# hpsim/OGL

Hardware: AMD Instinct MI355X
Metric: cg_iters_per_sec (higher is better)
Workload: dtype f64

## Files before the change

ogl_amd/csrc/kernels.hpp:

```cpp
#pragma once
#include <hip/hip_runtime.h>

#include "common.hpp"

namespace ogl {

struct DevCriterion {
    double tolerance, rel_tol;
    int32_t min_iter, max_iter, frequency, export_res;
};

struct DevScalars {
    double rho, prev_rho, beta;
    double alpha, omega, gamma;
    double norm_factor;
    double init_res, res;
    double xbar;
    double sums[4];
    int32_t iter;
    int32_t stop;
    int32_t n_evals;
    int32_t stop_phase;
    int32_t stop_turn;
    int32_t comm_error;
// ... 224 lines not shown
void launch_cg_rho_norm(hipStream_t st, int32_t n, const double *r, const double *inv_diag,
                        double *part_rho, double *part_norm, const DevScalars *gate);
void launch_cg_step1(hipStream_t st, int32_t n, double *p, const double *r, const double *inv_diag,
                     const DevScalars *s);
void launch_cg_step2(hipStream_t st, int32_t n, double *x, double *r, const double *p,
                     const double *q, const double *inv_diag, double *part_rho, double *part_norm,
                     const DevScalars *s);

struct HaloPutFused;
void launch_cg_step1x(hipStream_t st, int32_t n, double *p, double *x, const double *r,
                      const double *inv_diag, const DevScalars *s, const HaloPutFused *put = nullptr);
void launch_cg_step2r(hipStream_t st, int32_t n, double *r, const double *q, const double *inv_diag,
                      double *part_rho, double *part_norm, const DevScalars *s, double *z_out = nullptr,
                      const HaloPutFused *put = nullptr);

void launch_cg_step1x_fin(hipStream_t st, int32_t n, double *p, double *x, const double *r, const double *inv_diag,
                          const DevScalars *sin, DevScalars *sout, const double *part_rho,
                          const double *part_norm, double *history, int first, const LeadBox &lead = LeadBox{},
                          double *p_out = nullptr, const PRing &ring = PRing{});
void launch_cg_step2r_fin(hipStream_t st, int32_t n, double *r, const double *q, const double *inv_diag,
                          double *part_rho, double *part_norm, const DevScalars *sin, DevScalars *sout,
                          const double *part_beta, double *z_out = nullptr,
                          const LeadBox &lead = LeadBox{});
constexpr int FUSED_FIN_MAX_CHUNKS = 1024;
void launch_cg_turn_sym(hipStream_t st, const DevSym &A, const double *p_in, double *p_out, double *x, const double *z,
                        double *q, double *part_beta, const DevScalars *sin, DevScalars *sout,
                        const double *part_rho, const double *part_norm, double *history, int first,
                        const LeadBox &lead = LeadBox{});
void launch_cg_turn_sym_big(hipStream_t st, const DevSym &A, const double *p_in, double *p_out, double *x,
                            const double *z, double *q, double *part_beta, const DevScalars *s,
                            const HaloFused &hf = HaloFused{}, const double *p_halo_in = nullptr,
                            double *p_halo_out = nullptr);

void launch_gmres_mgs_fold(hipStream_t st, int32_t n, double *w, const double *vprev, double *h_out, const double *vdot,
                           const double *part_in, double *part_out, const DevScalars *gate, const LeadBox &lead = LeadBox{},
                           uint32_t tag = 0);
void launch_bicg_fold1(hipStream_t st, int32_t n, double *p, const double *r, const double *v, const double *inv_diag,
                       double *y, const DevScalars *sin, DevScalars *sout, const double *part_rho,
                       const double *part_norm, double *history, const LeadBox &lead = LeadBox{});
void launch_bicg_fold2(hipStream_t st, int32_t n, const double *r, const double *v, double *sv, const double *inv_diag,
                       double *z, double *part_norm_out, const DevScalars *sin, DevScalars *sout,
                       const double *part_beta, const LeadBox &lead = LeadBox{});
void launch_bicg_fold3(hipStream_t st, int32_t n, double *x, double *r, const double *sv, const double *t,
                       const double *y, const double *z, const double *rr, double *part_rho_out, double *part_norm_out,
                       const DevScalars *sin, DevScalars *sout, const double *part_gamma, const double *part_tt,
                       const double *part_snorm, double *history, int turn, const LeadBox &lead = LeadBox{});
// ... 107 lines not shown
```

ogl_amd/csrc/kernels_krylov.hip:

```cpp
#include "device_common.hpp"

namespace ogl {

namespace {

__global__ __launch_bounds__(BLOCK) void k_scale(int n, double *__restrict__ v, double f)
{
    const int i = blockIdx.x * BLOCK + threadIdx.x;
    if (i < n) v[i] = v[i] * f;
}

__global__ __launch_bounds__(BLOCK) void k_fill_xbar(int n, double *__restrict__ v,
                                                     const DevScalars *s)
{
    const int i = blockIdx.x * BLOCK + threadIdx.x;
    if (i < n) v[i] = s->xbar;
}

enum PartialOp { P_SUM = 0, P_DOT = 1, P_NORM1 = 2 };
template <int OP>
__global__ __launch_bounds__(BLOCK) void k_partials(int n, int n_chunks,
                                                    const double *__restrict__ a,
                                                    const double *__restrict__ b,
                                                    double *__restrict__ part,
// ... 480 lines not shown
        double2 vz = vrh;
        if (inv_diag) {
            vz.x = vrh.x * vi[h].x;
            vz.y = vrh.y * vi[h].y;
        }
        if (z_out) st2(z_out, rh, vz);
        double d = 0.0, a = 0.0;
        if (rh.n > 0) {
            d += vrh.x * vz.x;
            a += fabs(vrh.x);
        }
        if (rh.n > 1) {
            d += vrh.y * vz.y;
            a += fabs(vrh.y);
        }
        block_sum2(d, a, slot);
        if (threadIdx.x == 0) {
            part_rho[chunk] = d;
            part_norm[chunk] = a;
        }
    }
}

__global__ __launch_bounds__(BLOCK) void k_bicg_step1(int n, double *__restrict__ p,
                                                      const double *__restrict__ r,
                                                      const double *__restrict__ v,
                                                      const double *__restrict__ inv_diag,
                                                      double *__restrict__ y, const DevScalars *s)
{
    if (s->stop) return;
    const double rho = s->rho, prev = s->prev_rho, alpha = s->alpha, omega = s->omega;
    const RowPair rp = my_rows(blockIdx.x, n);
    const double2 vr = ld2_stream(r, rp);
    double2 vp = vr;
    if (prev * omega != 0.0) {
        const double tmp = rho / prev * alpha / omega;
        const double2 po = ld2_stream(p, rp), vv = ld2_stream(v, rp);
        vp.x = vr.x + tmp * (po.x - omega * vv.x);
        vp.y = vr.y + tmp * (po.y - omega * vv.y);
    }
    if (inv_diag) st2_stream(p, rp, vp); else st2(p, rp, vp);
    if (inv_diag) {
        const double2 vi = ld2_stream(inv_diag, rp);
        double2 vy;
        vy.x = vp.x * vi.x;
        vy.y = vp.y * vi.y;
// ... 847 lines not shown
    if (led) {
        OGL_STEP1X_K(true)
    } else {
        OGL_STEP1X(false, 0);
    }
#undef OGL_STEP1X_K
#undef OGL_STEP1X
}

constexpr int STEP2R_LEAD_CPW = 2;
void launch_cg_step2r_fin(hipStream_t st, int32_t n, double *r, const double *q, const double *inv_diag,
                          double *part_rho, double *part_norm, const DevScalars *sin, DevScalars *sout,
                          const double *part_beta, double *z_out, const LeadBox &lead)
{
    const int nc = (int)n_chunks(n);
    if (nc == 0) return;
    if (lead.box && nc >= 3 * FIN_WAVES)
        hipLaunchKernelGGL((k_cg_step2r_fin<true, STEP2R_LEAD_CPW>), dim3((nc + STEP2R_LEAD_CPW - 1) / STEP2R_LEAD_CPW),
                           dim3(BLOCK), 0, st, n, r, q, inv_diag, part_rho, part_norm, sin, sout, part_beta, nc, z_out, lead);
    else
        hipLaunchKernelGGL((k_cg_step2r_fin<false, 1>), dim3(nc), dim3(BLOCK), 0, st, n, r, q, inv_diag, part_rho, part_norm,
                           sin, sout, part_beta, nc, z_out, LeadBox{});
}

void launch_cg_step2(hipStream_t st, int32_t n, double *x, double *r, const double *p,
                     const double *q, const double *inv_diag, double *part_rho, double *part_norm,
                     const DevScalars *s)
{
    const int nc = (int)n_chunks(n);
    if (nc == 0) return;
    hipLaunchKernelGGL(k_cg_step2, dim3(nc), dim3(BLOCK), 0, st, n, x, r, p, q, inv_diag, part_rho,
                       part_norm, s);
}

void launch_bicg_step1(hipStream_t st, int32_t n, double *p, const double *r, const double *v,
                       const double *inv_diag, double *y, const DevScalars *s)
{
    const int nc = (int)n_chunks(n);
    if (nc == 0) return;
    hipLaunchKernelGGL(k_bicg_step1, dim3(nc), dim3(BLOCK), 0, st, n, p, r, v, inv_diag, y, s);
}

void launch_bicg_step2(hipStream_t st, int32_t n, const double *r, const double *v, double *sv,
                       const double *inv_diag, double *z, double *part_norm, const DevScalars *s)
{
    const int nc = (int)n_chunks(n);
// ... 174 lines not shown
```

ogl_amd/csrc/launch_key.hpp:

```cpp
#pragma once
#include <cstdint>
#include <cstring>
#include <type_traits>

#include "kernels.hpp"

namespace ogl {

struct KeyHasher {
    uint64_t h = 1469598103934665603ull;
    void bytes(const void *p, size_t n)
    {
        const unsigned char *c = static_cast<const unsigned char *>(p);
        for (size_t i = 0; i < n; ++i) h = (h ^ c[i]) * 1099511628211ull;
    }
    template <class T>
    std::enable_if_t<std::is_arithmetic<T>::value || std::is_pointer<T>::value || std::is_enum<T>::value> operator()(const T &v)
    {
        bytes(&v, sizeof(v));
    }
};

#define OGL_VIEW_FIELDS(T, n)                                                                                        \
    static_assert(sizeof(T) == n, "a field of " #T " was added, removed or resized: bring visit(KeyHasher &, const " #T \
// ... 11 lines not shown
    h(a.n_rows), h(a.width), h(a.stride), h(a.cols), h(a.vals), h(a.stream);
}
OGL_VIEW_FIELDS(DevSell, 112);
inline void visit(KeyHasher &h, const DevSell &a)
{
    h(a.n_rows), h(a.chunks), h(a.dict), h(a.codes), h(a.vals), h(a.spill_chunk_ptr), h(a.spill_rows), h(a.spill_ptrs);
    h(a.spill_cols), h(a.spill_vals), h(a.stream), h(a.xcd_group), h(a.rmap), h(a.block_order), h(a.n_blocks);
}
OGL_VIEW_FIELDS(DevSym, 64);
inline void visit(KeyHasher &h, const DevSym &a)
{
    h(a.n_rows), h(a.nd);
    for (int j = 0; j < 4; ++j) h(a.d[j]);
    h(a.mask), h(a.planes), h(a.stream), h(a.block_order), h(a.n_blocks);
}
OGL_VIEW_FIELDS(DevSymx, 96);
inline void visit(KeyHasher &h, const DevSymx &a)
{
    h(a.n_rows), h(a.chunks), h(a.chunks_general), h(a.n_blocks_general), h(a.mask), h(a.planes), h(a.ex_rowptr), h(a.ex_cols);
    h(a.ex_lrow), h(a.ex_vals), h(a.stream), h(a.fast), h(a.xcd_group), h(a.n_blocks);
}
OGL_VIEW_FIELDS(LeadBox, 24);
inline void visit(KeyHasher &h, const LeadBox &a) { h(a.box), h(a.timeout_ticks), h(a.early_loads); }

#undef OGL_VIEW_FIELDS

}
```

ogl_amd/csrc/solver.cpp:

```cpp
#include "solver_internal.hpp"

#include "setup_kernels.hpp"

#include <algorithm>
#include <atomic>
#include <chrono>
#include <condition_variable>
#include <cmath>
#include <cstddef>
#include <cstring>
#include <future>
#if defined(__x86_64__)
#include <immintrin.h>
#endif
#include <sched.h>
#include <mutex>
#include <thread>

using namespace ogl;


namespace {
#if defined(__x86_64__)
__attribute__((target("avx2"))) void stream_copy_avx2(char *d, const char *s, size_t len)
// ... 186 lines not shown
        (void)hipStreamSynchronize(comm_stream);
        stream_destroy(comm_stream);
        ev_destroy(ev_packed);
        ev_destroy(ev_received);
    }
    if (own_stream && stream) stream_destroy(stream);
}

void ogl_solver::drop_cg_graph()
{
    if (cg_graph) {
        (void)hipGraphExecDestroy(cg_graph);
        ledger::destroyed(ledger::GRAPH_EXEC);
    }
    cg_graph = nullptr;
    cg_graph_key = 0;
}

ogl_solver::~ogl_solver()
{
    drop_cg_graph();
    ledger::pinned_free(h_scal);
    ledger::dev_free(lead_box);
    for (auto &e : poll_ev)
        if (e) ev_destroy(e);
    for (auto &e : prof_ev)
        if (e) ev_destroy(e);
    for (auto &e : chk_ev)
        if (e) ev_destroy(e);
}

double ogl_solver::prop(const std::string &key, double dflt) const
{
    auto it = props.find(key);
    return it == props.end() ? dflt : it->second;
}

double ogl_solver::stream_above_bytes() const
{
    static const double env_default = [] {
        const char *e = std::getenv("OGL_STREAM_ABOVE_BYTES");
        return e ? atof(e) : STREAM_MATRIX_ABOVE_BYTES;
    }();
    return prop("streamAboveBytes", env_default);
}

// ... 988 lines not shown
```

ogl_amd/csrc/solver.hpp:

```cpp
#pragma once
#include <hip/hip_runtime.h>

#include <algorithm>
#include <map>
#include <memory>
#include <string>
#include <vector>

#include "comm.hpp"
#include "common.hpp"
#include "host_matrix.hpp"
#include "kernels.hpp"
#include "setup_kernels.hpp"
#include "spmv_layouts.hpp"

namespace ogl {

struct PrecondData {
    int kind = 0;
    size_t n_rows = 0;
    int stride = 0;
    int32_t n_blocks = 0;
    bool uniform_blocks = false;
    bool through_perm = false;
// ... 165 lines not shown
    ogl::DevBuf<double> d_p_halo;
    ogl::DevBuf<double> d_bj_tmp0, d_bj_tmp1;
    ogl::DevBuf<double> d_v, d_s, d_t, d_y, d_z, d_rr;
    ogl::DevBuf<double> d_V, d_gm;
    ogl::DevBuf<double> d_isai_tmp;
    ogl::DevBuf<double> d_fac_tmp[3];
    bool precond_ready = false;
    uint64_t precond_serial = 0, precond_pat = 0;
    bool precond_current() const;
    std::vector<int32_t> fac_seg_fwd, fac_seg_bwd;
    ogl::DevBuf<double> d_part0, d_part1, d_part2;
    int64_t band_order_rows = 0;
    bool source_diag_valid = false;
    int64_t csr_band_rows = 0;
    uint64_t csr_band_pat = 0;
    int csr_band(int64_t *band);
    ogl::DevBuf<int32_t> d_band_order;
    ogl::DevBuf<double> d_part3, d_part4, d_part5;
    ogl::DevBuf<ogl::DevScalars> d_scal;
    ogl::DevBuf<double> d_history;
    ogl::DevScalars *h_scal = nullptr;
    hipEvent_t poll_ev[2] = {nullptr, nullptr};
    unsigned long long *lead_box = nullptr;
    hipEvent_t chk_ev[2] = {nullptr, nullptr};
    bool x_resident = false, b_resident = false;
    ogl::PrecondData own_precond;
    const ogl::PrecondData *precond_data = nullptr;
    const double *precond = nullptr;

    std::map<std::string, double> props;

    std::vector<double> history;
    double t_update_matrix_ms = 0;
    std::vector<hipEvent_t> prof_ev;

    ~ogl_solver();

    int set_matrix(const ogl_ldu_view &ldu);
    int solve(const double *source, double *psi, ogl_perf *perf);
    int apply_resident(ogl_perf *perf);
    int upload_vec(ogl::DevBuf<double> &dst, const double *src);
    int ensure_vectors();
    int init_preconditioner();
    int generate_preconditioner(ogl::PrecondData &P);
    void apply_factor(const double *in, double *out, const ogl::DevScalars *gate, double *dot_part);
    int check_factor_breakdown(int32_t word);
    void apply_preconditioner(const double *in, double *out, const ogl::DevScalars *gate,
                              double *dot_part = nullptr);
    int dist_spmv(int mode, const double *x, const double *b, double *y, const ogl::SpmvDots &dots,
                  const ogl::DevScalars *gate, bool prepacked = false);
    void spmv_on(ogl::SpmvLayout l, int mode, const double *x, const double *b, double *y, const ogl::SpmvDots &dots,
                 const ogl::DevScalars *gate, const ogl::HaloFused &hf = ogl::HaloFused{});
    int finalize(int phase, ogl::FinArgs &a);
    int run_cg(ogl_perf *perf);
    int run_bicgstab(ogl_perf *perf);
    int run_krylov(ogl_perf *perf);
    struct KrylovRun;
    int krylov_plan(KrylovRun &k);
    int krylov_prepare(KrylovRun &k);
    int krylov_loop(KrylovRun &k);
    int krylov_enqueue(KrylovRun &k, int count);
    int krylov_finish(KrylovRun &k, ogl_perf *perf);
    int gmres_restart(KrylovRun &k, const ogl::DevScalars *gate);
    int gmres_update_x(KrylovRun &k, int cols, const ogl::DevScalars *gate);
    int turn_gmres(KrylovRun &k, int enq, int pe);
    int turn_cg_generic(KrylovRun &k, int enq, int pe);
    int turn_cg_generic_led(KrylovRun &k, int enq, int pe);
    int turn_cg_two_launch(KrylovRun &k, int enq, int pe);
    int turn_cg_three_launch(KrylovRun &k, int enq, int pe);
    int turn_cg_merged(KrylovRun &k, int enq, int pe);
    int turn_cg_five_launch(KrylovRun &k, int enq, int pe);
    int turn_bicg_folded(KrylovRun &k, int enq, int pe);
    int turn_bicg(KrylovRun &k, int enq, int pe);
    int time_spmv(int repeats, double *avg_ms);
    ogl::DevHalo halo() const;
    double prop(const std::string &key, double dflt) const;
    const ogl_solver *share_from = nullptr;
    const double *offdiag_upper = nullptr, *offdiag_lower = nullptr;
    uint64_t offdiag_sum = 0;
    bool offdiag_valid = false;
    const ogl_label *seen_lower_addr = nullptr, *seen_upper_addr = nullptr;
    ogl_label seen_faces = -1;
    struct SeenIface {
        const ogl_label *face_cells;
        ogl_label size, kind, neighb_proc, neighb_patch;
    };
    std::vector<SeenIface> seen_iface_cells;
    bool saw_addressing(const ogl_ldu_view &ldu) const;
    bool peer_safe_wait() const;
    double stream_above_bytes() const;
    double turn_extra_bytes() const;
    int32_t xcd_group() const;
// ... 3 lines not shown
```

ogl_amd/csrc/solver_krylov.cpp:

```cpp
#include "launch_key.hpp"
#include "solver_internal.hpp"

#include <algorithm>
#include <cmath>
#include <cstring>
#include <vector>

using namespace ogl;

HaloPutFused ogl_solver::begin_halo_put()
{
    HaloPutFused put;
    if (!(pat.non_local_nnz > 0 && peer_halo) || prop("haloFused", 1.0) == 0.0 || peer_safe_wait())
        return put;
    if (++halo_seq == 0) ++halo_seq;
    cur_halo = peer_halo_args(halo_seq);
    put.P = cur_halo;
    put.chunk_sptr = d_chunk_sptr.p;
    put.send_pos = d_send_pos.p;
    put.send_idxs = d_send_idxs.p;
    put.ticket = d_ticket.p;
    put.n_put_chunks = n_put_chunks;
    return put;
}
// ... 128 lines not shown
    int cur = 0;
    bool bicg = false, gmres = false, generic = false, multi = false;
    bool fused = false, fused2 = false, merged = false, merged_halo = false, bicg_fold = false, gmres_fold = false;
    int m = 0;
    int64_t ldv = 0;
    double n_global = 0.0;
    size_t n_halo = 0;
    double *p0 = nullptr, *p1 = nullptr, *ph = nullptr;
    double *z_kept = nullptr;
    LeadBox lead{};
    uint32_t lead_tag = 0;
    DevCriterion crit{};
    bool is_final = false;
    int max_checks = 0, max_turns = 0;
    int prof_stride = 0, prof_cap = 0;
    hipEvent_t ev_chk[2] = {nullptr, nullptr};
    double t_start = 0.0;
    FinArgs fg{}, chk{}, f1{}, f2{};
    const double *beta_ptr = nullptr;
    double *gm = nullptr, *gm_y = nullptr;
    double *y = nullptr, *z = nullptr;
    int enq = 0;
    double *gm_h(int i, int j) const { return gm + (size_t)j * (m + 1) + i; }
    PRing ring{};
    double *p_of_turn(int turn) const
    {
        if (ring.k > 0) return ring.b[turn % ring.k];
        return (merged && (turn & 1)) ? p1 : p0;
    }
    PRing ring_of_turn(int turn) const
    {
        PRing r = ring;
        r.phase = ring.k > 0 ? turn % ring.k : 0;
        return r;
    }
    double *p_halo_of_turn(int turn) const { return ph + (size_t)(turn & 1) * n_halo; }
    bool gmres_scale_late() const { return gmres && !generic && has_diag; }
    bool has_diag = false;
    bool folded() const { return fused || bicg_fold; }
};

int ogl_solver::run_cg(ogl_perf *perf) { return run_krylov(perf); }
int ogl_solver::run_bicgstab(ogl_perf *perf) { return run_krylov(perf); }

int ogl_solver::run_krylov(ogl_perf *perf)
{
// ... 74 lines not shown
    DevScalars *s = k.s;
    const bool bicg = k.bicg, gmres = k.gmres, generic = k.generic, merged = k.merged;
    int ring_k = 0;
    if (k.lead.box != nullptr && k.fused && !k.fused2 && prop("deferX2", 1.0) != 0.0) {
        const double want = prop("deferX", 2.0);
        ring_k = want >= 8.0 ? 8 : want >= 4.0 ? 4 : want >= 2.0 ? 2 : 0;
    }
    props["deferXInUse"] = (double)ring_k;
    props["deferX2InUse"] = ring_k ? 1.0 : 0.0;
    if (merged || ring_k) OGL_TRY(d_p2.alloc((size_t)n + 2, st));
    for (int i = 2; i < ring_k; ++i) OGL_TRY(d_pring[i - 2].alloc((size_t)n + 2, st));
    if (merged && precond) OGL_TRY(d_z.alloc((size_t)n + 2, st));
    k.n_halo = (size_t)pat.non_local_nnz;
    if (k.merged_halo) {
        OGL_TRY(d_p_halo.alloc(2 * k.n_halo + 2, st));
        OGL_HIP_CHECK(hipMemsetAsync(d_p_halo.p, 0, d_p_halo.n * sizeof(double), st));
    }
    k.p0 = d_p.p;
    k.p1 = d_p2.p;
    k.ring.k = ring_k;
    for (int i = 0; i < ring_k; ++i) k.ring.b[i] = i == 0 ? d_p.p : i == 1 ? d_p2.p : d_pring[i - 2].p;
    k.ph = d_p_halo.p;
    k.z_kept = merged && precond ? d_z.p : nullptr;

    k.is_final = cfg.rel_tol == 0.0;
    const int prev_iters = (int)prop(k.is_final ? "prevSolveIters_final" : "prevSolveIters", 1);
    const double prev_cost = prop("_prev_solve", 0.0);
    DevCriterion &crit = k.crit;
    crit.tolerance = cfg.tolerance;
    crit.rel_tol = cfg.rel_tol;
    crit.max_iter = bicg ? 2 * cfg.max_iter : cfg.max_iter;
    crit.export_res = cfg.export_res;
    ogl_host_adapt_criterion(&cfg, prev_iters, prev_cost, &crit.min_iter, &crit.frequency);
    if (crit.frequency < 1) return fail(OGL_ERR_INVALID, "evalFrequency must be >= 1");
    k.max_checks = std::max(crit.max_iter, crit.min_iter) + crit.frequency + 1;
    k.max_turns = bicg ? k.max_checks / 2 + 1 : k.max_checks;
    OGL_TRY(d_history.alloc((size_t)std::max(k.max_checks, crit.max_iter + std::max(1, cfg.norm_eval_limit) + 1) + 4, st));
    if (cfg.export_res)
        OGL_HIP_CHECK(hipMemsetAsync(d_history.p, 0, d_history.n * sizeof(double), st));
    if (k.bicg_fold) {
        OGL_TRY(d_part3.alloc((size_t)nc, st));
        OGL_TRY(d_part4.alloc((size_t)nc, st));
        OGL_TRY(d_part5.alloc((size_t)nc, st));
    }
    if (bicg) {
        const size_t nv = (size_t)n + 2;
// ... 232 lines not shown
    if (enq == 0) OGL_HIP_CHECK(hipEventRecord(k.ev_chk[0], st));
    if (pe >= 0) OGL_HIP_CHECK(hipEventRecord(prof_ev[2 * pe], st));
    launch_cg_turn_sym(st, sym(), k.p_of_turn(enq), k.p_of_turn(enq + 1), d_x.p, k.z_kept ? k.z_kept : d_r.p,
                       d_q.p, d_part2.p, k.s, k.s2, d_part0.p, d_part1.p, d_history.p, enq == 0 ? 1 : 0, k.lead);
    if (pe >= 0) OGL_HIP_CHECK(hipEventRecord(prof_ev[2 * pe + 1], st));
    if (enq == 0) OGL_HIP_CHECK(hipEventRecord(k.ev_chk[1], st));
    launch_cg_step2r_fin(st, k.n, d_r.p, d_q.p, precond, d_part0.p, d_part1.p, k.s2, k.s, d_part2.p, k.z_kept, k.lead);
    return OGL_OK;
}

int ogl_solver::turn_cg_three_launch(KrylovRun &k, int enq, int pe)
{
    hipStream_t st = k.st;
    const int n = k.n;
    if (enq == 0) OGL_HIP_CHECK(hipEventRecord(k.ev_chk[0], st));
    double *p_new = k.p_of_turn(enq + 1);
    launch_cg_step1x_fin(st, n, k.p_of_turn(enq), d_x.p, d_r.p, precond, k.s, k.s2, d_part0.p, d_part1.p, d_history.p,
                         enq == 0 ? 1 : 0, k.lead, p_new, k.ring_of_turn(enq));
    if (enq == 0) OGL_HIP_CHECK(hipEventRecord(k.ev_chk[1], st));
    if (pe >= 0) OGL_HIP_CHECK(hipEventRecord(prof_ev[2 * pe], st));
    OGL_TRY(dist_spmv(SPMV_PLAIN, p_new, nullptr, d_q.p, SpmvDots{p_new, d_part2.p, nullptr}, k.s2));
    if (pe >= 0) OGL_HIP_CHECK(hipEventRecord(prof_ev[2 * pe + 1], st));
    launch_cg_step2r_fin(st, n, d_r.p, d_q.p, precond, d_part0.p, d_part1.p, k.s2, k.s, d_part2.p, nullptr, k.lead);
    return OGL_OK;
}

int ogl_solver::turn_cg_merged(KrylovRun &k, int enq, int pe)
{
    hipStream_t st = k.st;
    const int n = k.n;
    DevScalars *s = k.s;
    if (pe >= 0) OGL_HIP_CHECK(hipEventRecord(prof_ev[2 * pe], st));
    if (k.merged_halo) {
        launch_cg_turn_sym_big(st, sym(), k.p_of_turn(enq), k.p_of_turn(enq + 1), d_x.p,
                               k.z_kept ? k.z_kept : d_r.p, d_q.p, d_part0.p, s,
                               halo_fused_args(cur_halo), k.p_halo_of_turn(enq), k.p_halo_of_turn(enq + 1));
    } else {
        launch_cg_turn_sym_big(st, sym(), k.p_of_turn(enq), k.p_of_turn(enq + 1), d_x.p,
                               k.z_kept ? k.z_kept : d_r.p, d_q.p, d_part0.p, s);
    }
    if (pe >= 0) OGL_HIP_CHECK(hipEventRecord(prof_ev[2 * pe + 1], st));
    OGL_TRY(finalize(FIN_BETA, k.f1));
    if (k.merged_halo) {
        const HaloPutFused put = begin_halo_put();
        launch_cg_step2r(st, n, d_r.p, d_q.p, precond, d_part0.p, d_part1.p, s, k.z_kept, &put);
    } else {
// ... 82 lines not shown
                          SpmvDots{d_s.p, d_part0.p, d_part1.p}, s));
        OGL_TRY(finalize(FIN_BICG_OMEGA, f2));
    }
    launch_bicg_step3(st, n, d_x.p, d_r.p, d_s.p, d_t.p, y, z, d_rr.p, d_part0.p,
                      d_part1.p, s, enq);
    OGL_TRY(finalize(FIN_CG_CHECK, k.chk));
    return OGL_OK;
}

int ogl_solver::krylov_enqueue(KrylovRun &k, int count)
{
    for (int i = 0; i < count; ++i, ++k.enq) {
        const int enq = k.enq;
        const bool prof = k.prof_stride && enq % k.prof_stride == 0 && enq / k.prof_stride < k.prof_cap;
        const int pe = prof ? enq / k.prof_stride : -1;
        if (k.gmres)
            OGL_TRY(turn_gmres(k, enq, pe));
        else if (k.bicg)
            OGL_TRY(k.bicg_fold ? turn_bicg_folded(k, enq, pe) : turn_bicg(k, enq, pe));
        else if (k.generic)
            OGL_TRY(k.fused ? turn_cg_generic_led(k, enq, pe) : turn_cg_generic(k, enq, pe));
        else if (k.fused2)
            OGL_TRY(turn_cg_two_launch(k, enq, pe));
        else if (k.fused)
            OGL_TRY(turn_cg_three_launch(k, enq, pe));
        else if (k.merged)
            OGL_TRY(turn_cg_merged(k, enq, pe));
        else
            OGL_TRY(turn_cg_five_launch(k, enq, pe));
    }
    return OGL_OK;
}

int ogl_solver::krylov_loop(KrylovRun &k)
{
    hipStream_t st = k.st;
    const bool fused = k.fused;
    auto poll_record = [&](int slot) -> int {
        OGL_HIP_CHECK(hipMemcpyAsync(&h_scal[slot], k.bicg_fold ? k.slot_s[k.cur] : k.s, sizeof(DevScalars),
                                     hipMemcpyDeviceToHost, st));
        OGL_HIP_CHECK(hipEventRecord(poll_ev[slot], st));
        return OGL_OK;
    };

    const int batch = k.bicg ? 8 : 16;

    const bool graphable = !k.gmres && !k.bicg && !k.generic && !k.multi && k.prof_cap == 0 &&
                           prop("hipGraph", fused ? 1.0 : 0.0) != 0.0;
    auto enqueue_turns = [&](int count) -> int {
        if (!graphable || count != batch || (fused && k.enq == 0)) return krylov_enqueue(k, count);
        KeyHasher kh;
        kh(k.n), kh(batch), kh(cfg.matrix_format), kh(spmv_layout);
        kh(k.fused), kh(k.fused2), kh(k.merged), kh(k.ring.k), kh(k.p0), kh(k.p1), kh(k.z_kept), kh(k.s), kh(k.s2), kh(pat_id);
        for (const void *v : {(const void *)d_p.p, (const void *)d_x.p, (const void *)d_r.p, (const void *)d_q.p,
                              (const void *)precond, (const void *)d_part0.p, (const void *)d_part1.p,
                              (const void *)d_part2.p, (const void *)d_history.p, (const void *)d_z.p, (const void *)d_p2.p})
            kh(v);
        for (int i = 0; i < k.ring.k; ++i) kh((const void *)k.ring.b[i]);
        visit(kh, csr());
        switch (spmv_layout) {
        case SpmvLayout::Ell: visit(kh, ell()); break;
        case SpmvLayout::Sell: visit(kh, sell()); break;
        case SpmvLayout::Sym: visit(kh, sym()); break;
        case SpmvLayout::Symx: visit(kh, symx()); break;
        default: break;
        }
        visit(kh, k.lead);
        const uint64_t key = kh.h;
        if (!cg_graph || key != cg_graph_key) {
            if (cg_graph) {
                (void)hipGraphExecDestroy(cg_graph);
                ledger::destroyed(ledger::GRAPH_EXEC);
            }
            cg_graph = nullptr;
            OGL_HIP_CHECK(hipStreamBeginCapture(st, hipStreamCaptureModeThreadLocal));
            const int before = k.enq;
            const int rc = krylov_enqueue(k, batch);
            k.enq = before;
            hipGraph_t g = nullptr;
            const hipError_t e = hipStreamEndCapture(st, &g);
            if (rc != OGL_OK || e != hipSuccess) {
                if (g) (void)hipGraphDestroy(g);
                return rc != OGL_OK ? rc : fail(OGL_ERR_HIP, "stream capture failed: %s", hipGetErrorString(e));
            }
            const hipError_t ei = hipGraphInstantiate(&cg_graph, g, nullptr, nullptr, 0);
            (void)hipGraphDestroy(g);
            if (ei != hipSuccess) {
                cg_graph = nullptr;
                return fail(OGL_ERR_HIP, "hipGraphInstantiate failed: %s", hipGetErrorString(ei));
            }
// ... 7 lines not shown
    };
    OGL_TRY(enqueue_turns(std::min(batch, k.max_turns - k.enq)));
    OGL_TRY(poll_record(0));
    for (int j = 0;; ++j) {
        const bool more = k.enq < k.max_turns;
        if (more) {
            OGL_TRY(enqueue_turns(std::min(batch, k.max_turns - k.enq)));
            OGL_TRY(poll_record((j + 1) & 1));
        }
        OGL_HIP_CHECK(hipEventSynchronize(poll_ev[j & 1]));
        if (h_scal[j & 1].stop) break;
        if (!more && k.folded()) break;
        if (!more) return fail(OGL_ERR_STATE, "criterion did not stop within maxIter + frequency");
    }
    return OGL_OK;
}

int ogl_solver::krylov_finish(KrylovRun &k, ogl_perf *perf)
{
    hipStream_t st = k.st;
    const int n = k.n, m = k.m;
    DevScalars *s = k.s, *s2 = k.s2;
    const bool bicg = k.bicg, gmres = k.gmres, fused = k.fused, bicg_fold = k.bicg_fold;
    if (fused)
        launch_cg_step1x_fin(st, n, k.p_of_turn(k.enq), d_x.p, k.generic ? d_z.p : d_r.p, k.generic ? nullptr : precond, s, s2,
                             d_part0.p, d_part1.p, d_history.p, 0, k.lead, k.p_of_turn(k.enq + 1), k.ring_of_turn(k.enq));
    if (bicg_fold) {
        launch_bicg_fold1(st, n, d_p.p, d_r.p, d_v.p, precond, k.y, k.slot_s[k.cur], k.slot_s[k.cur ^ 1], d_part0.p,
                          d_part1.p, d_history.p, k.lead);
        k.cur ^= 1;
    }
    DevScalars *fin_s = bicg_fold ? k.slot_s[k.cur] : (fused ? s2 : s);
    if (precond_data && precond_data->factor())
        OGL_HIP_CHECK(hipMemcpyAsync(&fin_s->factor_breakdown, precond_data->f_breakdown.p, sizeof(int32_t),
                                     hipMemcpyDeviceToDevice, st));
    OGL_HIP_CHECK(hipStreamSynchronize(st));
    OGL_HIP_CHECK(hipGetLastError());
    DevScalars fin;
    OGL_HIP_CHECK(hipMemcpy(&fin, fin_s, sizeof(fin), hipMemcpyDeviceToHost));
    OGL_TRY(check_factor_breakdown(fin.factor_breakdown));
    if (k.folded() && !fin.stop) return fail(OGL_ERR_STATE, "criterion did not stop within maxIter + frequency");
    if (fin.comm_error && !k.multi && k.lead.box)
        return fail(OGL_ERR_STATE, "leader finalisation timed out: the sums of a turn were not published within "
                    "leadTimeoutS = %g s (check %d)", prop("leadTimeoutS", 10.0), fin.iter);
    if (fin.comm_error)
        return fail(OGL_ERR_COMM, "peer all-reduce timed out: a rank did not take part (check %d)",
                    fin.iter);
    if (fin.x_pending) {
        launch_cg_step1x(st, n, k.p_of_turn(k.enq), d_x.p, d_r.p, precond, s);
        OGL_HIP_CHECK(hipStreamSynchronize(st));
        OGL_HIP_CHECK(hipGetLastError());
    }
    if (gmres) {
        const int steps = fin.iter - 1;
        const int cols = steps <= 0 ? 0 : (steps - 1) % m + 1;
        OGL_TRY(gmres_update_x(k, cols, nullptr));
        OGL_HIP_CHECK(hipStreamSynchronize(st));
        OGL_HIP_CHECK(hipGetLastError());
    }
    const double t_solve = now_ms() - k.t_start;
    history.clear();
    if (cfg.export_res) {
        history.resize(fin.iter);
        OGL_HIP_CHECK(hipMemcpy(history.data(), d_history.p, (size_t)fin.iter * sizeof(double),
                                hipMemcpyDeviceToHost));
    }
    float chk_ms = 0.f;
    OGL_HIP_CHECK(hipEventElapsedTime(&chk_ms, k.ev_chk[0], k.ev_chk[1]));

    props["haloWaits"] = (double)fin.halo_waits;
    props["haloWaitUs"] = (double)fin.halo_wait_ticks / 100.0;
    props["allreduceWaits"] = (double)fin.reduce_waits;
    props["allreduceWaitUs"] = (double)fin.reduce_wait_ticks / 100.0;
    props["peerSafeWaitInUse"] = (pat.non_local_nnz > 0 && peer_halo && peer_safe_wait()) ? 1.0 : 0.0;
    props["peerSharedDevice"] = reg->peer_shared_device ? 1.0 : 0.0;
    perf->initial_residual = fin.init_res;
    perf->final_residual = fin.res;
    perf->n_iterations = bicg ? fin.iter / 2 : fin.iter;
    perf->n_norm_evals = fin.n_evals;
    perf->norm_factor = fin.norm_factor;
    perf->t_solve_ms = t_solve;
    const int turns_done = bicg ? fin.iter / 2 : std::max(0, fin.iter - 1);
    perf->spmv_avg_ms = 0;
    perf->spmv_launches = 0;
    if (k.prof_cap) {
        double acc = 0;
        const int cnt = std::min((turns_done + k.prof_stride - 1) / k.prof_stride, k.prof_cap);
        for (int i = 0; i < cnt; ++i) {
            float ms = 0.f;
            OGL_HIP_CHECK(hipEventElapsedTime(&ms, prof_ev[2 * i], prof_ev[2 * i + 1]));
            acc += ms;
        }
// ... 103 lines not shown
```

Baseline: 4408.

## Fuse CG residual update and p/x update into one persistent held-z kernel

Result: faster. 4669 (median of 6 runs) (+5.9%).

```diff
diff --git a/ogl_amd/csrc/kernels.hpp b/ogl_amd/csrc/kernels.hpp
--- a/ogl_amd/csrc/kernels.hpp
+++ b/ogl_amd/csrc/kernels.hpp
@@ -270,6 +270,16 @@
                           double *part_rho, double *part_norm, const DevScalars *sin, DevScalars *sout,
                           const double *part_beta, double *z_out = nullptr,
                           const LeadBox &lead = LeadBox{});
+struct HeldZ {
+    unsigned long long *tagged = nullptr;
+    int32_t grid = 0;
+    int32_t x_early = 1;
+};
+int held_z_grid(int *chunks_per_workgroup);
+int launch_resident_census(hipStream_t st, int grid, unsigned *arrived, int *out, long long timeout_ticks);
+void launch_cg_step2r1x(hipStream_t st, int32_t n, double *r, const double *q, const double *inv_diag, double *p,
+                        double *p_out, double *x, DevScalars *s, const double *part_beta, double *history,
+                        const LeadBox &lead, const PRing &ring, const HeldZ &hz);
 constexpr int FUSED_FIN_MAX_CHUNKS = 1024;
 void launch_cg_turn_sym(hipStream_t st, const DevSym &A, const double *p_in, double *p_out, double *x, const double *z,
                         double *q, double *part_beta, const DevScalars *sin, DevScalars *sout,
diff --git a/ogl_amd/csrc/kernels_krylov.hip b/ogl_amd/csrc/kernels_krylov.hip
--- a/ogl_amd/csrc/kernels_krylov.hip
+++ b/ogl_amd/csrc/kernels_krylov.hip
@@ -526,6 +526,258 @@
     }
 }
 
+__device__ __forceinline__ void put_tagged(unsigned long long *w, uint32_t tag, double v)
+{
+    const unsigned long long bits = (unsigned long long)__double_as_longlong(v);
+    __hip_atomic_store(w, ((unsigned long long)tag << 32) | (uint32_t)bits, __ATOMIC_RELAXED, LEAD_SCOPE);
+    __hip_atomic_store(w + 1, ((unsigned long long)tag << 32) | (uint32_t)(bits >> 32), __ATOMIC_RELAXED, LEAD_SCOPE);
+}
+
+__device__ __forceinline__ void lead_wave_sums_tagged(const LeadBox &L, uint32_t tag, const unsigned long long *tagged,
+                                                      int m, int w, int array)
+{
+    constexpr int Q = 4;
+    if (threadIdx.x >= WAVE) return;
+    const int lane = threadIdx.x;
+    const long long t0 = wall_clock64();
+    double s = 0.0;
+    bool arrived = true;
+    for (long i0 = w * WAVE + lane; arrived && i0 < m; i0 += (long)FIN_BLOCK * Q) {
+        unsigned long long lo[Q], hi[Q];
+        for (;;) {
+            bool all = true;
+#pragma unroll
+            for (int e = 0; e < Q; ++e) {
+                const long i = i0 + (long)FIN_BLOCK * e;
+                lo[e] = hi[e] = (unsigned long long)tag << 32;
+                if (i < m) {
+                    lo[e] = __hip_atomic_load(tagged + 4 * i + 2 * array, __ATOMIC_RELAXED, LEAD_SCOPE);
+                    hi[e] = __hip_atomic_load(tagged + 4 * i + 2 * array + 1, __ATOMIC_RELAXED, LEAD_SCOPE);
+                }
+            }
+#pragma unroll
+            for (int e = 0; e < Q; ++e) all = all && (uint32_t)(lo[e] >> 32) == tag && (uint32_t)(hi[e] >> 32) == tag;
+            if (all) break;
+            if (wall_clock64() - t0 > L.timeout_ticks) {
+                arrived = false;
+                break;
+            }
+            __builtin_amdgcn_s_sleep(1);
+        }
+#pragma unroll
+        for (int e = 0; e < Q; ++e)
+            if (i0 + (long)FIN_BLOCK * e < m) s += __longlong_as_double((long long)((hi[e] << 32) | (uint32_t)lo[e]));
+    }
+    if (!__all(arrived)) return;
+    s = wave_sum(s);
+    if (lane < LEAD_REPLICAS) put_tagged(L.box + (size_t)lane * LEAD_REPLICA_STRIDE + array * 2 * FIN_WAVES + 2 * w, tag, s);
+}
+
+template <int R, int L, int B, int K>
+__global__ __launch_bounds__(BLOCK, B) void k_cg_step2r1x(int n, double *__restrict__ r, const double *__restrict__ q,
+                                                          const double *__restrict__ inv_diag, double *p, double *p_out,
+                                                          double *__restrict__ x, DevScalars *s,
+                                                          const double *__restrict__ part_beta,
+                                                          unsigned long long *tagged, int n_part, double *history,
+                                                          LeadBox lead, const double *p_pend, int ring_phase,
+                                                          int x_early)
+{
+    static_assert(K == 0 || K == 2, "p in place or two p buffers");
+    constexpr int D = 2;
+    __shared__ double zl[L > 0 ? L * CHUNK_ROWS : 1];
+    __shared__ double sh[4];
+    __shared__ int sh_stop;
+    __shared__ double slot[2 * N_WAVES];
+    __shared__ double lead_words[LEAD_BOX_WORDS / 2];
+    __shared__ int lead_timed_out;
+    static_assert(L * CHUNK_ROWS >= LEAD_STAGE, "the leaders of beta stage through zl, which is idle until phase 1");
+    const uint32_t seq = s->launch_seq;
+    lead_leaders<1>(lead, seq, part_beta, nullptr, nullptr, n_part, zl);
+    const int stopped = s->stop;
+    const double s_rho = s->rho, s_nf = s->norm_factor, s_init = s->init_res;
+    const int phase = K > 0 ? ring_phase : 0;
+    const bool defers = K > 0 && phase != 0;
+    const unsigned s_pending = K > 0 ? (unsigned)s->defer_valid : 0u;
+    const double s_t1 = K > 0 ? s->t_ring[1] : 0.0;
+    const int s_iter = s->iter, s_evals = s->n_evals;
+    const double c_tol = s->crit.tolerance, c_rel = s->crit.rel_tol;
+    const int c_min = s->crit.min_iter, c_max = s->crit.max_iter, c_freq = s->crit.frequency, c_exp = s->crit.export_res;
+    const int G = gridDim.x, w = blockIdx.x, tx = threadIdx.x;
+    const int mine = w < n_part ? (n_part - w + G - 1) / G : 0;
+    double2 fr[D], fq[D], fi[D];
+    auto ask = [&](int i, int d) {
+        const RowPair rp = my_rows(w + i * G, n);
+        fr[d] = ld2(r, rp);
+        fq[d] = ld2_stream(q, rp);
+        fi[d].x = fi[d].y = 1.0;
+        if (inv_diag) fi[d] = ld2_stream(inv_diag, rp);
+    };
+#pragma unroll
+    for (int d = 0; d < D; ++d) ask(d, d);
+    if (stopped) return;
+    if (!lead_wait(lead, 2 * FIN_WAVES, seq, lead_words, &lead_timed_out)) {
+        if (tx == 0) s->comm_error = s->stop = 1;
+        return;
+    }
+    if (tx == 0) sh[0] = lead_total(lead_words, 0);
+    __syncthreads();
+    const double beta = sh[0];
+    const uint32_t tag = seq + 1;
+    double2 zr[R];
+#pragma unroll
+    for (int i = 0; i < R + L; ++i) {
+        if (i >= mine) continue;
+        const int chunk = w + i * G;
+        const RowPair rp = my_rows(chunk, n);
+        double2 vr = fr[i % D];
+        const double2 vq = fq[i % D], vi = fi[i % D];
+        if (i + D < R + L) ask(i + D, i % D);
+        if (beta != 0.0) {
+            const double t = s_rho / beta;
+            vr.x -= t * vq.x;
+            vr.y -= t * vq.y;
+            st2(r, rp, vr);
+        }
+        double2 vz = vr;
+        if (inv_diag) {
+            vz.x = vr.x * vi.x;
+            vz.y = vr.y * vi.y;
+        }
+        if (i < R) {
+            zr[i < R ? i : 0] = vz;
+        } else {
+            zl[(i - R) * CHUNK_ROWS + ROWS_PER_THREAD * tx] = vz.x;
+            zl[(i - R) * CHUNK_ROWS + ROWS_PER_THREAD * tx + 1] = vz.y;
+        }
+        double d = 0.0, a = 0.0;
+        if (rp.n > 0) {
+            d += vr.x * vz.x;
+            a += fabs(vr.x);
+        }
+        if (rp.n > 1) {
+            d += vr.y * vz.y;
+            a += fabs(vr.y);
+        }
+        block_sum2(d, a, slot);
+        if (tx == 0) {
+            put_tagged(tagged + 4 * (size_t)chunk, tag, d);
+            put_tagged(tagged + 4 * (size_t)chunk + 2, tag, a);
+        }
+    }
+    if (w < 2 * FIN_WAVES) lead_wave_sums_tagged(lead, tag, tagged, n_part, w % FIN_WAVES, w / FIN_WAVES);
+    const bool own_term = beta != 0.0;
+    const double t_own = own_term ? s_rho / beta : 0.0;
+    auto update_x = [&](const RowPair &rp, const double2 &vp, int upto) {
+        const bool pend = K > 1 && 1 < upto && ((s_pending >> 1) & 1u);
+        if (!pend && !own_term) return;
+        double2 vx = ld2_stream(x, rp);
+        if (pend) {
+            const double2 v1 = ld2(p_pend, rp);
+            vx.x += s_t1 * v1.x;
+            vx.y += s_t1 * v1.y;
+        }
+        if (own_term) {
+            vx.x += t_own * vp.x;
+            vx.y += t_own * vp.y;
+        }
+        st2_stream(x, rp, vx);
+    };
+    const bool early = x_early != 0 && !defers;
+    if (early) {
+#pragma unroll 2
+        for (int i = 0; i < mine; ++i) {
+            const RowPair rp = my_rows(w + i * G, n);
+            update_x(rp, ld2(p, rp), K);
+        }
+    }
+    if (!lead_wait(lead, 4 * FIN_WAVES, tag, lead_words, &lead_timed_out)) {
+        if (tx == 0) s->comm_error = s->stop = 1;
+        return;
+    }
+    if (tx == 0) {
+        const double prev_rho = s_rho, rho = lead_total(lead_words, 0), norm = lead_total(lead_words, 1);
+        int iter = s_iter, n_evals = s_evals, stop = 0;
+        double init_res = s_init, res = 0.0;
+        bool evaluated = false;
+        if (iter > 0 && iter < c_min) {
+            iter += 1;
+        } else if (iter % c_freq != 0) {
+            iter += 1;
+        } else {
+            evaluated = true;
+            n_evals += 1;
+            res = norm;
+            if (iter == 0) init_res = res / s_nf;
+            res /= s_nf;
+            if (c_exp && history && w == 0) history[iter] = res;
+            if (iter >= c_max) stop = 1;
+            if (res < c_tol) stop = 1;
+            if (c_rel > 0 && res < c_rel * init_res) stop = 1;
+            iter += 1;
+        }
+        sh[1] = prev_rho;
+        sh[2] = rho;
+        sh_stop = stop;
+        if (w == 0) {
+            s->beta = beta;
+            s->prev_rho = prev_rho;
+            s->rho = rho;
+            s->iter = iter;
+            s->x_pending = 0;
+            if (evaluated) {
+                s->n_evals = n_evals;
+                s->init_res = init_res;
+                s->res = res;
+            }
+            if (stop) s->stop = 1;
+            s->launch_seq = seq + 2;
+            s->defer_valid = (defers && !stop) ? (int)(s_pending | (own_term ? 1u << phase : 0u)) : 0;
+            if (defers && own_term) s->t_ring[phase] = t_own;
+        }
+    }
+    __syncthreads();
+    const double prev = sh[1], rho = sh[2];
+    const int stop = sh_stop;
+    const double tmp = (prev == 0.0) ? 0.0 : rho / prev;
+#pragma unroll
+    for (int i = 0; i < R + L; ++i) {
+        if (i >= mine) continue;
+        const RowPair rp = my_rows(w + i * G, n);
+        double2 vp = ld2(p, rp);
+        if (!defers && !early) update_x(rp, vp, K);
+        if (defers && stop) update_x(rp, vp, phase);
+        if (stop) continue;
+        double2 vz;
+        if (i < R) {
+            vz = zr[i < R ? i : 0];
+        } else {
+            vz.x = zl[(i - R) * CHUNK_ROWS + ROWS_PER_THREAD * tx];
+            vz.y = zl[(i - R) * CHUNK_ROWS + ROWS_PER_THREAD * tx + 1];
+        }
+        vp.x = vz.x + tmp * vp.x;
+        vp.y = vz.y + tmp * vp.y;
+        st2(p_out, rp, vp);
+    }
+}
+
+template <int B>
+__global__ __launch_bounds__(BLOCK, B) void k_resident_census(unsigned *arrived, int *out, long long timeout_ticks)
+{
+    extern __shared__ double census_lds[];
+    if (threadIdx.x == 0) {
+        census_lds[0] = 0.0;
+        atomicAdd(arrived, 1u);
+        const long long t0 = wall_clock64();
+        while (__hip_atomic_load(arrived, __ATOMIC_RELAXED, __HIP_MEMORY_SCOPE_AGENT) < gridDim.x) {
+            if (wall_clock64() - t0 > timeout_ticks) {
+                *out = 1;
+                break;
+            }
+            __builtin_amdgcn_s_sleep(8);
+        }
+    }
+}
+
 __global__ __launch_bounds__(BLOCK) void k_bicg_step1(int n, double *__restrict__ p,
                                                       const double *__restrict__ r,
                                                       const double *__restrict__ v,
@@ -1419,6 +1671,47 @@
         hipLaunchKernelGGL((k_cg_step2r_fin<false, 1>), dim3(nc), dim3(BLOCK), 0, st, n, r, q, inv_diag, part_rho, part_norm,
                            sin, sout, part_beta, nc, z_out, LeadBox{});
 }
+
+constexpr int HZ_B = 4, HZ_R = 11, HZ_L = 9;
+#define OGL_HELD_Z(K) k_cg_step2r1x<HZ_R, HZ_L, HZ_B, K>
+
+int held_z_grid(int *chunks_per_workgroup)
+{
+    *chunks_per_workgroup = HZ_R + HZ_L;
+    int dev = 0, per_cu[2] = {0, 0};
+    hipDeviceProp_t prop;
+    if (hipGetDevice(&dev) != hipSuccess || hipGetDeviceProperties(&prop, dev) != hipSuccess) return 0;
+    if (hipOccupancyMaxActiveBlocksPerMultiprocessor(&per_cu[0], OGL_HELD_Z(0), BLOCK, 0) != hipSuccess ||
+        hipOccupancyMaxActiveBlocksPerMultiprocessor(&per_cu[1], OGL_HELD_Z(2), BLOCK, 0) != hipSuccess)
+        return 0;
+    return prop.multiProcessorCount * std::min(HZ_B, std::min(per_cu[0], per_cu[1]));
+}
+
+int launch_resident_census(hipStream_t st, int grid, unsigned *arrived, int *out, long long timeout_ticks)
+{
+    hipFuncAttributes fa;
+    if (hipFuncGetAttributes(&fa, reinterpret_cast<const void *>(OGL_HELD_Z(2))) != hipSuccess) return 1;
+    if (hipMemsetAsync(arrived, 0, sizeof(unsigned), st) != hipSuccess || hipMemsetAsync(out, 0, sizeof(int), st) != hipSuccess)
+        return 1;
+    hipLaunchKernelGGL((k_resident_census<HZ_B>), dim3(grid), dim3(BLOCK), fa.sharedSizeBytes, st, arrived, out,
+                       timeout_ticks);
+    return 0;
+}
+
+void launch_cg_step2r1x(hipStream_t st, int32_t n, double *r, const double *q, const double *inv_diag, double *p,
+                        double *p_out, double *x, DevScalars *s, const double *part_beta, double *history,
+                        const LeadBox &lead, const PRing &ring, const HeldZ &hz)
+{
+    const int nc = (int)n_chunks(n);
+    if (nc == 0) return;
+    if (ring.k == 2)
+        hipLaunchKernelGGL((OGL_HELD_Z(2)), dim3(hz.grid), dim3(BLOCK), 0, st, n, r, q, inv_diag, p, p_out, x, s, part_beta,
+                           hz.tagged, nc, history, lead, ring.b[1], ring.phase, hz.x_early);
+    else
+        hipLaunchKernelGGL((OGL_HELD_Z(0)), dim3(hz.grid), dim3(BLOCK), 0, st, n, r, q, inv_diag, p, p, x, s, part_beta,
+                           hz.tagged, nc, history, lead, nullptr, 0, hz.x_early);
+}
+#undef OGL_HELD_Z
 
 void launch_cg_step2(hipStream_t st, int32_t n, double *x, double *r, const double *p,
                      const double *q, const double *inv_diag, double *part_rho, double *part_norm,
diff --git a/ogl_amd/csrc/launch_key.hpp b/ogl_amd/csrc/launch_key.hpp
--- a/ogl_amd/csrc/launch_key.hpp
+++ b/ogl_amd/csrc/launch_key.hpp
@@ -57,6 +57,8 @@
 }
 OGL_VIEW_FIELDS(LeadBox, 24);
 inline void visit(KeyHasher &h, const LeadBox &a) { h(a.box), h(a.timeout_ticks), h(a.early_loads); }
+OGL_VIEW_FIELDS(HeldZ, 16);
+inline void visit(KeyHasher &h, const HeldZ &a) { h(a.tagged), h(a.grid), h(a.x_early); }
 
 #undef OGL_VIEW_FIELDS
 
diff --git a/ogl_amd/csrc/solver.cpp b/ogl_amd/csrc/solver.cpp
--- a/ogl_amd/csrc/solver.cpp
+++ b/ogl_amd/csrc/solver.cpp
@@ -232,6 +232,7 @@
     drop_cg_graph();
     ledger::pinned_free(h_scal);
     ledger::dev_free(lead_box);
+    ledger::dev_free(held_z_box);
     for (auto &e : poll_ev)
         if (e) ev_destroy(e);
     for (auto &e : prof_ev)
diff --git a/ogl_amd/csrc/solver.hpp b/ogl_amd/csrc/solver.hpp
--- a/ogl_amd/csrc/solver.hpp
+++ b/ogl_amd/csrc/solver.hpp
@@ -211,6 +211,9 @@
     ogl::DevScalars *h_scal = nullptr;
     hipEvent_t poll_ev[2] = {nullptr, nullptr};
     unsigned long long *lead_box = nullptr;
+    unsigned long long *held_z_box = nullptr;
+    size_t held_z_words = 0;
+    int held_z_census = 0, held_z_census_grid = 0;
     hipEvent_t chk_ev[2] = {nullptr, nullptr};
     bool x_resident = false, b_resident = false;
     ogl::PrecondData own_precond;
@@ -257,6 +260,8 @@
     int turn_cg_generic_led(KrylovRun &k, int enq, int pe);
     int turn_cg_two_launch(KrylovRun &k, int enq, int pe);
     int turn_cg_three_launch(KrylovRun &k, int enq, int pe);
+    int turn_cg_held_z(KrylovRun &k, int enq, int pe);
+    int plan_held_z(KrylovRun &k);
     int turn_cg_merged(KrylovRun &k, int enq, int pe);
     int turn_cg_five_launch(KrylovRun &k, int enq, int pe);
     int turn_bicg_folded(KrylovRun &k, int enq, int pe);
diff --git a/ogl_amd/csrc/solver_krylov.cpp b/ogl_amd/csrc/solver_krylov.cpp
--- a/ogl_amd/csrc/solver_krylov.cpp
+++ b/ogl_amd/csrc/solver_krylov.cpp
@@ -174,6 +174,8 @@
     double *y = nullptr, *z = nullptr;
     int enq = 0;
     double *gm_h(int i, int j) const { return gm + (size_t)j * (m + 1) + i; }
+    HeldZ hz{};
+    bool held_z() const { return hz.grid > 0; }
     PRing ring{};
     double *p_of_turn(int turn) const
     {
@@ -294,6 +296,7 @@
     for (int i = 0; i < ring_k; ++i) k.ring.b[i] = i == 0 ? d_p.p : i == 1 ? d_p2.p : d_pring[i - 2].p;
     k.ph = d_p_halo.p;
     k.z_kept = merged && precond ? d_z.p : nullptr;
+    OGL_TRY(plan_held_z(k));
 
     k.is_final = cfg.rel_tol == 0.0;
     const int prev_iters = (int)prop(k.is_final ? "prevSolveIters_final" : "prevSolveIters", 1);
@@ -572,6 +575,79 @@
     OGL_TRY(dist_spmv(SPMV_PLAIN, p_new, nullptr, d_q.p, SpmvDots{p_new, d_part2.p, nullptr}, k.s2));
     if (pe >= 0) OGL_HIP_CHECK(hipEventRecord(prof_ev[2 * pe + 1], st));
     launch_cg_step2r_fin(st, n, d_r.p, d_q.p, precond, d_part0.p, d_part1.p, k.s2, k.s, d_part2.p, nullptr, k.lead);
+    return OGL_OK;
+}
+
+int ogl_solver::turn_cg_held_z(KrylovRun &k, int enq, int pe)
+{
+    hipStream_t st = k.st;
+    const int n = k.n;
+    double *p_new = k.p_of_turn(enq + 1);
+    if (enq == 0) {
+        OGL_HIP_CHECK(hipEventRecord(k.ev_chk[0], st));
+        launch_cg_step1x_fin(st, n, k.p_of_turn(0), d_x.p, d_r.p, precond, k.s, k.s2, d_part0.p, d_part1.p, d_history.p, 1,
+                             k.lead, p_new, k.ring_of_turn(0));
+        OGL_HIP_CHECK(hipEventRecord(k.ev_chk[1], st));
+    }
+    if (pe >= 0) OGL_HIP_CHECK(hipEventRecord(prof_ev[2 * pe], st));
+    OGL_TRY(dist_spmv(SPMV_PLAIN, p_new, nullptr, d_q.p, SpmvDots{p_new, d_part2.p, nullptr}, k.s2));
+    if (pe >= 0) OGL_HIP_CHECK(hipEventRecord(prof_ev[2 * pe + 1], st));
+    launch_cg_step2r1x(st, n, d_r.p, d_q.p, precond, p_new, k.p_of_turn(enq + 2), d_x.p, k.s2, d_part2.p, d_history.p, k.lead,
+                       k.ring_of_turn(enq + 1), k.hz);
+    return OGL_OK;
+}
+
+int ogl_solver::plan_held_z(KrylovRun &k)
+{
+    k.hz = HeldZ{};
+    props["heldZInUse"] = 0.0;
+    if (!(k.lead.box != nullptr && k.fused && !k.fused2 && !k.generic && !k.multi && (k.ring.k == 0 || k.ring.k == 2)))
+        return OGL_OK;
+    bool streams = false;
+    switch (spmv_layout) {
+    case SpmvLayout::Ell: streams = ell().stream; break;
+    case SpmvLayout::Sell: streams = sell().stream; break;
+    case SpmvLayout::Sym: streams = sym().stream; break;
+    case SpmvLayout::Symx: streams = symx().stream; break;
+    default: streams = csr().stream; break;
+    }
+    if (prop("heldZ", streams ? 1.0 : 0.0) == 0.0 || held_z_census < 0) return OGL_OK;
+    int per_wg = 0;
+    int grid = held_z_grid(&per_wg);
+    grid = std::min(grid, (int)prop("heldZGrid", (double)grid));
+    if (grid < 2 * 16) return OGL_OK;
+    const double cap = std::min((double)grid * per_wg, prop("heldZMaxChunks", (double)grid * per_wg));
+    if ((double)k.nc > cap) return OGL_OK;
+    hipStream_t st = k.st;
+    const size_t words = 4 * (size_t)k.nc;
+    if (!held_z_box || held_z_words < words) {
+        ledger::dev_free(held_z_box);
+        held_z_box = nullptr;
+        void *b = nullptr;
+        OGL_HIP_CHECK(ledger::dev_malloc(&b, words * sizeof(unsigned long long), true));
+        held_z_box = static_cast<unsigned long long *>(b);
+        held_z_words = words;
+    }
+    OGL_HIP_CHECK(hipMemsetAsync(held_z_box, 0, held_z_words * sizeof(unsigned long long), st));
+    if (held_z_census == 0 || held_z_census_grid < grid) {
+        void *c = nullptr;
+        OGL_HIP_CHECK(ledger::dev_malloc(&c, 2 * sizeof(int)));
+        int timed_out = 1;
+        const int rc = launch_resident_census(st, grid, static_cast<unsigned *>(c), static_cast<int *>(c) + 1,
+                                              (long long)(prop("heldZCensusS", 1.0) * 1e8));
+        hipError_t e = rc == 0 ? hipMemcpyAsync(&timed_out, static_cast<int *>(c) + 1, sizeof(int), hipMemcpyDeviceToHost, st)
+                               : hipErrorUnknown;
+        if (e == hipSuccess) e = hipStreamSynchronize(st);
+        ledger::dev_free(c);
+        if (e != hipSuccess) return fail(OGL_ERR_HIP, "census of the held-z grid failed: %s", hipGetErrorString(e));
+        held_z_census = timed_out ? -1 : 1;
+        held_z_census_grid = grid;
+        if (timed_out) return OGL_OK;
+    }
+    k.hz.tagged = held_z_box;
+    k.hz.grid = grid;
+    k.hz.x_early = prop("heldZEarlyX", 1.0) != 0.0 ? 1 : 0;
+    props["heldZInUse"] = 1.0;
     return OGL_OK;
 }
 
@@ -700,6 +776,8 @@
             OGL_TRY(k.fused ? turn_cg_generic_led(k, enq, pe) : turn_cg_generic(k, enq, pe));
         else if (k.fused2)
             OGL_TRY(turn_cg_two_launch(k, enq, pe));
+        else if (k.held_z())
+            OGL_TRY(turn_cg_held_z(k, enq, pe));
         else if (k.fused)
             OGL_TRY(turn_cg_three_launch(k, enq, pe));
         else if (k.merged)
@@ -715,7 +793,7 @@
     hipStream_t st = k.st;
     const bool fused = k.fused;
     auto poll_record = [&](int slot) -> int {
-        OGL_HIP_CHECK(hipMemcpyAsync(&h_scal[slot], k.bicg_fold ? k.slot_s[k.cur] : k.s, sizeof(DevScalars),
+        OGL_HIP_CHECK(hipMemcpyAsync(&h_scal[slot], k.bicg_fold ? k.slot_s[k.cur] : (k.held_z() ? k.s2 : k.s), sizeof(DevScalars),
                                      hipMemcpyDeviceToHost, st));
         OGL_HIP_CHECK(hipEventRecord(poll_ev[slot], st));
         return OGL_OK;
@@ -744,6 +822,7 @@
         default: break;
         }
         visit(kh, k.lead);
+        visit(kh, k.hz);
         const uint64_t key = kh.h;
         if (!cg_graph || key != cg_graph_key) {
             if (cg_graph) {
@@ -797,7 +876,7 @@
     const int n = k.n, m = k.m;
     DevScalars *s = k.s, *s2 = k.s2;
     const bool bicg = k.bicg, gmres = k.gmres, fused = k.fused, bicg_fold = k.bicg_fold;
-    if (fused)
+    if (fused && !k.held_z())
         launch_cg_step1x_fin(st, n, k.p_of_turn(k.enq), d_x.p, k.generic ? d_z.p : d_r.p, k.generic ? nullptr : precond, s, s2,
                              d_part0.p, d_part1.p, d_history.p, 0, k.lead, k.p_of_turn(k.enq + 1), k.ring_of_turn(k.enq));
     if (bicg_fold) {
@@ -843,6 +922,7 @@
     float chk_ms = 0.f;
     OGL_HIP_CHECK(hipEventElapsedTime(&chk_ms, k.ev_chk[0], k.ev_chk[1]));
 
+    props["turnsEnqueued"] = (double)k.enq;
     props["haloWaits"] = (double)fin.halo_waits;
     props["haloWaitUs"] = (double)fin.halo_wait_ticks / 100.0;
     props["allreduceWaits"] = (double)fin.reduce_waits;
```
